# zehuichen123/Graph-DETR4D

Measured on AMD Instinct MI355X. Metric: decoder_samples_per_sec_900q_T4, higher is better.
Workload: dtype f32 (bf16x3 GEMMs)

## Files before the change

graph-detr4d_amd/_lib.py:

```python
import ctypes
import os
import threading

from . import switches

_HERE = os.path.dirname(os.path.abspath(__file__))
LIB_PATH = switches.path('GD4D_LIB_PATH') or os.path.join(_HERE, 'libgd4d.so')
ABI_VERSION = 56
PIXEL_MAJOR, HEAD_MAJOR = 0, 1

F32, BF16, F16 = 0, 1, 2
GATHER_REVERSED = 0x100

_c = ctypes
_vp, _i, _f = _c.c_void_p, _c.c_int, _c.c_float

SIGNATURES = {
    'gd4d_abi_version': (_i, []),
    'gd4d_error_string': (_c.c_char_p, [_i]),
    'gd4d_last_hip_error': (_c.c_char_p, []),
    'gd4d_trace_enable': (_i, [_vp]),
    'gd4d_cross_attn_fwd': (_i, [_vp, _vp, _vp, _vp, _vp, _vp, _vp, _vp, _f, _f, _vp, _vp, _vp,
                                 _i, _i, _i, _i, _i, _i, _i, _i, _i, _i, _vp, _vp]),
    'gd4d_pyramid_channels_last_fwd': (_i, [_vp, _vp, _vp, _i, _i, _i, _i, _i, _i, _vp]),
    'gd4d_cross_attn_agg_fwd': (_i, [_vp] * 8 + [_f, _f] + [_vp] * 4 + [_i] * 9 + [_vp] * 5),
    'gd4d_cross_attn_plan_bytes': (_c.c_size_t, [_i] * 5),
    'gd4d_cross_attn_plan_fwd': (_i, [_vp] * 6 + [_f, _f, _vp, _vp, _c.c_int64, _vp, _c.c_size_t, _vp, _vp, _vp] + [_i] * 7 + [_vp, _vp]),
    'gd4d_cross_attn_agg_sliced_fwd': (_i, [_vp, _c.c_int64, _vp, _vp] + [_i] * 8 + [_vp, _i, _i, _vp]),
    'gd4d_cross_attn_agg_items_fwd': (_i, [_vp, _vp, _vp, _c.c_int64, _c.c_int64, _vp, _vp, _vp] + [_i] * 8 + [_vp, _i, _i, _vp]),
    'gd4d_cross_attn_agg_items_coarse_fwd': (_i, [_vp, _vp, _vp, _c.c_int64, _c.c_int64, _vp, _vp, _vp, _vp, _vp, _vp] + [_i] * 8 + [_vp, _vp]),
    'gd4d_gather_slice_group': (_i, [_i]),
    'gd4d_gather_slice_group_get': (_i, []),
    'gd4d_gather_walk': (_i, [_i, _i, _i, _i, _vp, _vp]),
    'gd4d_gather_walk_dir': (_i, [_i, _i, _i, _i, _i, _vp, _vp]),
    'gd4d_chain_guest_bytes': (_c.c_size_t, []),
    'gd4d_value_proj_image_bytes': (_c.c_size_t, []),
    'gd4d_value_proj_image': (_i, [_vp, _vp, _vp, _vp]),
    'gd4d_value_proj_guest_fwd': (_i, [_vp, _i, _vp]),
    'gd4d_row_chain_guest_fwd': (_i, [_vp, _i, _vp, _i, _i, _vp, _vp]),
    'gd4d_row_chain_choice': (_i, [_vp, _i, _vp, _i, _i]),
    'gd4d_row_chain_choice_name': (_c.c_char_p, [_i]),
    'gd4d_row_chain_specialise': (_i, [_i]),
    'gd4d_row_chain_fill_fwd': (_i, [_vp, _i, _vp, _i, _i, _vp, _i, _vp, _vp, _i, _i, _i, _i, _i, _vp]),
    'gd4d_cross_attn_agg_items_count_fwd': (_i, [_vp, _vp, _vp, _c.c_int64, _c.c_int64, _vp, _vp, _vp] + [_i] * 8 + [_vp, _vp, _vp, _vp, _c.c_size_t, _vp]),
    'gd4d_pyramid_slice_planar_fwd': (_i, [_vp, _vp, _vp, _i, _i, _i, _i, _i, _i, _vp]),
    'gd4d_value_proj_heads_fwd': (_i, [_vp] * 5 + [_i, _i, _i, _vp]),
    'gd4d_value_proj_heads_bwd': (_i, [_vp] * 5 + [_i, _i, _i, _vp]),
    'gd4d_value_proj_heads_bwd_weight_workspace_bytes': (_c.c_size_t, []),
    'gd4d_value_proj_heads_bwd_weight': (_i, [_vp] * 6 + [_c.c_size_t, _i, _i, _i, _i, _vp]),
    'gd4d_value_proj_heads_bwd_weight_group': (_i, [_vp] * 6 + [_i, _vp, _c.c_size_t, _i, _i, _i, _vp]),
    'gd4d_cross_attn_dot_bytes': (_c.c_size_t, [_i] * 5),
    'gd4d_cross_attn_dot_sliced': (_i, [_vp, _c.c_int64, _vp, _vp, _vp, _c.c_size_t] + [_i] * 8 + [_vp, _vp]),
    'gd4d_cross_attn_dot_sliced_wgrad': (_i, [_vp, _c.c_int64, _vp, _vp, _vp, _c.c_size_t] + [_i] * 8 + [_vp] + [_vp] * 5 + [_i, _i, _vp]),
    'gd4d_cross_attn_plan_bwd': (_i, [_vp] * 6 + [_f, _f] + [_vp] * 9 + [_c.c_size_t, _vp] + [_i] * 7 + [_vp, _vp]),
    'gd4d_pyramid_grad_chunks': (_c.c_int64, [_vp, _i, _i]),
    'gd4d_pyramid_grad_slots_bytes': (_c.c_size_t, [_i] * 5),
    'gd4d_pyramid_grad_count': (_i, [_vp, _vp, _vp, _c.c_int64, _vp, _vp, _c.c_size_t] + [_i] * 6 + [_vp]),
    'gd4d_pyramid_grad_scan_workspace_bytes': (_c.c_size_t, [_c.c_int64]),
    'gd4d_pyramid_grad_scan': (_i, [_vp, _vp, _vp, _c.c_size_t, _c.c_int64, _vp]),
    'gd4d_pyramid_grad_fill': (_i, [_vp, _vp, _vp, _vp, _c.c_uint32, _vp] + [_i] * 5 + [_vp]),
    'gd4d_pyramid_grad_chunk_geometry': (_i, [_vp, _i, _i, _vp]),
    'gd4d_pyramid_grad_sort': (_i, [_vp] * 5 + [_c.c_int64, _vp]),
    'gd4d_pyramid_grad_reduce': (_i, [_vp] * 7 + [_i, _i, _i, _i, _vp]),
    'gd4d_query_order_fwd': (_i, [_vp, _vp, _vp, _i, _i, _vp]),
    'gd4d_refine_reference_order_fwd': (_i, [_vp, _vp, _vp, _vp, _vp, _i, _i, _i, _vp]),
    'gd4d_cross_attn_bwd': (_i, [_vp] * 8 + [_f, _f] + [_vp] * 6 + [_i] * 10 + [_vp, _vp, _c.c_size_t, _vp]),
    'gd4d_cross_attn_bwd_workspace_bytes': (_c.c_size_t, [_i] * 5),
    'gd4d_detr3d_fwd': (_i, [_vp, _vp, _vp, _vp, _vp, _vp, _f, _f, _vp, _vp, _vp,
# ... 220 lines not shown
```

graph-detr4d_amd/csrc/gd4d_cross_attn_sliced.hip:

```cpp
#include <stdlib.h>

#include <type_traits>

#include "gd4d_common.h"
#include "gd4d_cross_attn_shared.h"
#include "gd4d_cross_attn_sliced.h"
#include "gd4d_pyramid_count.h"

namespace gd4d {

GD4D_TRACE_UNIT(sliced)


struct PlanParams {
  CrossAttnParams c;
  PyramidGeom g;
  int* hdr;
  uint2* pair;
  int cap_t;
  float4* item;
  int cap_i;
  int both;
};

// ... 286 lines not shown
  if (grp - k * period == ca.every && k < ca.groups) {
    pyramid_grad_count_body(ca.hdr, ca.pair, ca.cap_t, HH, ca.BQ, ca.g, ca.count, ca.slots,
                            (k * 8 + (int)(blockIdx.x & 7)) * HH + (int)(threadIdx.x >> 6));
    return;
  }
  int pos, sl;
  if (!sliced_walk(ip.s, (int)blockIdx.x - 8 * min(k, ca.groups), pos, sl)) return;
  cross_attn_agg_items_body<HH, LT, VT, false>(ip, pos, sl, s_raw);
}

struct SpParams {
  const float* in[GD4D_MAX_LEVELS];
  int hw[GD4D_MAX_LEVELS];
  int start[GD4D_MAX_LEVELS];
  int tiles[GD4D_MAX_LEVELS];
  int tile_base[GD4D_MAX_LEVELS + 1];
  void* out;
  int R, L, S, total;
};

constexpr int SP_PX = 64, SP_C = 256, SP_PITCH = 260, SP_THREADS = 512;
constexpr int SP_LDS = 84 * 1024;

template <bool OUT_BF16>
__device__ __forceinline__ void sp_store4(void* base, size_t elem, float4 v) {
  if (OUT_BF16) {
    uint2 pk;
    pk.x = (unsigned)f32_to_bf16(v.x) | ((unsigned)f32_to_bf16(v.y) << 16);
    pk.y = (unsigned)f32_to_bf16(v.z) | ((unsigned)f32_to_bf16(v.w) << 16);
    *reinterpret_cast<uint2*>(static_cast<uint16_t*>(base) + elem) = pk;
  } else {
    *reinterpret_cast<float4*>(static_cast<float*>(base) + elem) = v;
  }
}

template <bool OUT_BF16, bool PERSISTENT>
__global__ __launch_bounds__(SP_THREADS) void pyramid_slice_planar_kernel(const SpParams p) {
  extern __shared__ __attribute__((aligned(16))) float s_tp[];
  const int tid = threadIdx.x, lane = tid & 63, wave = tid >> 6;
  trace_mark(g_trace_sliced, 4ull);
  float v[32];
  int npx = 0, ostart = 0, pix0 = 0, row = 0;
  auto load_tile = [&](int t) {
    const float* src = p.in[0];
    int hw = p.hw[0], tiles = p.tiles[0], tbase = 0, os = p.start[0];
#pragma unroll
// ... 11 lines not shown
  int t = blockIdx.x;
  if (t < p.total) load_tile(t);
  const size_t plane = (size_t)p.R * p.S * kSlice;
  while (t < p.total) {
    const int c_npx = npx, c_ostart = ostart, c_pix0 = pix0, c_row = row;
#pragma unroll
    for (int i = 0; i < 32; ++i) s_tp[lane * SP_PITCH + wave * 32 + i] = v[i];
    __syncthreads();
    const int tn = t + gridDim.x;
    if (PERSISTENT && tn < p.total) load_tile(tn);
    const size_t obase = (size_t)wave * plane + ((size_t)c_row * p.S + c_ostart + c_pix0) * kSlice;
#pragma unroll
    for (int i = 0; i < SP_PX / 8; ++i) {
      const int px = 8 * i + (lane >> 3);
      if (px < c_npx)
        sp_store4<OUT_BF16>(p.out, obase + (size_t)px * kSlice + (lane & 7) * 4,
                            *reinterpret_cast<const float4*>(&s_tp[px * SP_PITCH + wave * 32 + (lane & 7) * 4]));
    }
    if (!PERSISTENT) break;
    __syncthreads();
    t = tn;
  }
  trace_mark(g_trace_sliced, 0x84ull);
}

}

extern "C" void gd4d_trace_set_sliced(unsigned long long* p) { gd4d::trace_set_sliced(p); }

extern "C" size_t gd4d_cross_attn_plan_bytes(int B, int N, int Q, int Hh, int P) {
  if (B <= 0 || N <= 0 || Q <= 0 || Hh <= 0 || P <= 0) return 0;
  const size_t pairs = (size_t)B * Q * Hh * gd4d::plan_cap_t(N, P) * 64 * sizeof(uint2);
  return gd4d::plan_hdr_bytes(B, Q) + pairs;
}

namespace gd4d {
static int fill_plan_params(PlanParams& pp, const float* ref, const float* offsets, const float* attn_logits,
                            const float* cam_logits, const float* lidar2img, const double* pc_range, float img_h, float img_w,
                            const int32_t* level_hw, const int64_t* cam_stride_bytes, int64_t pix_stride_bytes, void* plan,
                            size_t plan_bytes, float* wsum, uint8_t* mask_out, float* uv_out, int B, int N, int Q, int Hh, int L, int P,
                            int flags, const int32_t* query_order);
}

extern "C" int gd4d_cross_attn_plan_fwd(const float* ref, const float* offsets, const float* attn_logits,
                                        const float* cam_logits, const float* lidar2img, const double* pc_range,
                                        float img_h, float img_w, const int32_t* level_hw, const int64_t* cam_stride_bytes,
// ... 309 lines not shown
extern "C" int gd4d_cross_attn_agg_items_count_fwd(const void* const* level_ptrs, const int32_t* level_hw,
                                                   const int64_t* cam_stride_bytes, int64_t pix_stride_bytes,
                                                   int64_t slice_stride_bytes, const void* plan_items, float* agg, float* wsum, int B,
                                                   int N, int Q, int Hh, int C, int L, int P, int feats_dtype,
                                                   const int32_t* query_order, const void* plan_pairs, int32_t* count, void* slots,
                                                   size_t slots_bytes, void* stream) {
  using namespace gd4d;
  if (!plan_pairs || !count || !slots || !level_hw || !cam_stride_bytes) return GD4D_EINVAL;
  if (B <= 0 || N <= 0 || Q <= 0 || Hh <= 0 || L <= 0) return GD4D_EINVAL;
  if ((P != kPoints && P != 8) || L > 4 || N > 64 || B > 16 || Hh > kPlanHdr) return GD4D_EUNSUPPORTED;
  if (slots_bytes < (size_t)B * Q * Hh * plan_cap_t(N, P) * 64 * sizeof(uint2)) return GD4D_EWORKSPACE;
  CountArgs ca{};
  if (int rc = fill_chunks(ca.g, level_hw, cam_stride_bytes, pix_stride_bytes, B * N, L)) return rc;
  ca.hdr = static_cast<const int*>(plan_pairs);
  ca.pair = reinterpret_cast<const uint2*>(static_cast<const char*>(plan_pairs) + plan_hdr_bytes(B, Q));
  ca.count = count;
  ca.slots = static_cast<uint2*>(slots);
  ca.cap_t = plan_cap_t(N, P);
  ca.BQ = B * Q;
  return items_fwd_impl(level_ptrs, level_hw, cam_stride_bytes, pix_stride_bytes, slice_stride_bytes, plan_items, agg, wsum, B, N, Q, Hh,
                        C, L, P, feats_dtype, query_order, 0, 8, stream, &ca);
}

extern "C" int gd4d_pyramid_slice_planar_fwd(const void* const* feats, const int32_t* level_hw, void* out, int R, int C,
                                             int L, int in_dtype, int out_dtype, int max_cus, void* stream) {
  using namespace gd4d;
  if (!feats || !level_hw || !out || R <= 0 || C <= 0 || L <= 0) return GD4D_EINVAL;
  if (C != SP_C || L > GD4D_MAX_LEVELS || in_dtype != GD4D_F32) return GD4D_EUNSUPPORTED;
  if (out_dtype != GD4D_F32 && out_dtype != GD4D_BF16) return GD4D_EUNSUPPORTED;
  if (!aligned16(out)) return GD4D_EALIGN;
  SpParams p{};
  int s = 0, base = 0;
  for (int l = 0; l < L; ++l) {
    if (!feats[l] || level_hw[2 * l] <= 0 || level_hw[2 * l + 1] <= 0) return GD4D_EINVAL;
    const int hw = level_hw[2 * l] * level_hw[2 * l + 1];
    p.in[l] = static_cast<const float*>(feats[l]); p.hw[l] = hw; p.start[l] = s; p.tiles[l] = (hw + SP_PX - 1) / SP_PX;
    p.tile_base[l] = base;
    s += hw;
    base += R * p.tiles[l];
  }
  for (int l = L; l <= GD4D_MAX_LEVELS; ++l) p.tile_base[l] = base;
  for (int l = L; l < GD4D_MAX_LEVELS; ++l) { p.tiles[l] = 1; p.hw[l] = 1; }
  p.out = out; p.R = R; p.L = L; p.S = s; p.total = base;
  hipStream_t st = static_cast<hipStream_t>(stream);
  const bool ob = out_dtype == GD4D_BF16;
  const size_t tile_lds = (size_t)SP_PX * SP_PITCH * sizeof(float);
  auto go = [&](auto kern, int blocks, size_t lds) -> int {
    if (!allow_dynamic_lds(reinterpret_cast<const void*>(kern), (int)lds)) return GD4D_ELAUNCH;
    hipLaunchKernelGGL(kern, dim3(blocks), dim3(SP_THREADS), lds, st, p);
    return check_launch();
  };
  if (max_cus > 0) {
    const int blocks = max_cus < base ? max_cus : base;
    return ob ? go(pyramid_slice_planar_kernel<true, true>, blocks, SP_LDS) : go(pyramid_slice_planar_kernel<false, true>, blocks, SP_LDS);
  }
  return ob ? go(pyramid_slice_planar_kernel<true, false>, base, tile_lds) : go(pyramid_slice_planar_kernel<false, false>, base, tile_lds);
}
```

graph-detr4d_amd/csrc/gd4d_request.hip:

```cpp
#include <string.h>

#include <new>
#include <vector>

#include "gd4d_common.h"

namespace {

struct Step {
  gd4d_request_step s;
  std::vector<gd4d_chain_op> prog_a, prog_b;
  gd4d_chain_guest guest;
  std::vector<gd4d_request_patch> patches;
  std::vector<uint64_t> table[GD4D_REQ_TABLES];
};

bool is_chain(int kind) { return kind == GD4D_REQ_ROW_CHAIN || kind == GD4D_REQ_ROW_CHAIN2 || kind == GD4D_REQ_ROW_CHAIN_GUEST; }

struct Shape {
  const char* name;
  int ptrs, tables;
};

const Shape* shape_of(int kind) {
  static const Shape shapes[] = {
      {nullptr, 0, 0},
      {"gd4d_row_chain_fwd", 0, 0},
      {"gd4d_row_chain2_fwd", 0, 0},
      {"gd4d_row_chain_guest_fwd", 0, 0},
      {"gd4d_mha_core_fwd", 5, 0},
      {"gd4d_mha_core_presplit_fwd", 5, 0},
      {"gd4d_cross_attn_plan_fwd", 10, 3},
      {"gd4d_cross_attn_agg_items_coarse_fwd", 5, 5},
      {"gd4d_cross_attn_agg_items_fwd", 4, 3},
      {"gd4d_cross_attn_agg_sliced_fwd", 3, 1},
      {"gd4d_pyramid_slice_planar_fwd", 1, 2},
      {"gd4d_value_proj_guest_fwd", 0, 0},
      {"gd4d_query_order_fwd", 2, 1},
      {"hipEventRecord", 0, 0},
      {"hipStreamWaitEvent", 0, 0},
      {"hipMemcpyAsync", 2, 0},
  };
  if (kind < GD4D_REQ_ROW_CHAIN || kind > GD4D_REQ_COPY) return nullptr;
  return &shapes[kind];
}

int64_t table_need(const gd4d_request_step& s, int k) {
  const int64_t L = s.kind == GD4D_REQ_SLICE_PLANAR ? s.i[2] : s.kind == GD4D_REQ_PLAN ? s.i[4] : s.i[5];
  switch (s.kind) {
    case GD4D_REQ_PLAN: return k == 0 ? 48 : k == 1 ? 8 * L : 8 * L;
    case GD4D_REQ_AGG_COARSE: return k == 0 ? 8 * L : k == 1 ? 8 * L : k == 2 ? 8 * L : 16;
    case GD4D_REQ_AGG_ITEMS: return 8 * L;
    case GD4D_REQ_AGG_SLICED: return 8 * L;
    case GD4D_REQ_SLICE_PLANAR: return 8 * L;
    case GD4D_REQ_QUERY_ORDER: return 48;
  }
  return 0;
}

}

struct gd4d_decoder_request {
  std::vector<Step> steps;
  std::vector<hipEvent_t> events;
  hipEvent_t join = nullptr;
  int nbindings = 0;
  bool uses_side = false;
};

namespace {

int validate(const gd4d_request_step* steps, int nsteps, int nbindings) {
  if (steps == nullptr || nsteps <= 0 || nsteps > GD4D_REQ_MAX_STEPS || nbindings < 0) return GD4D_EINVAL;
  bool recorded[GD4D_REQ_MAX_EVENTS] = {};
  for (int n = 0; n < nsteps; ++n) {
    const gd4d_request_step& s = steps[n];
    const Shape* sh = shape_of(s.kind);
    if (sh == nullptr || (s.side != 0 && s.side != 1) || s.npatches < 0 || (s.npatches > 0 && s.patches == nullptr)) return GD4D_EINVAL;
    for (int k = 0; k < sh->ptrs; ++k)
      if (s.p[k].binding >= nbindings) return GD4D_EINVAL;
    if (s.kind == GD4D_REQ_PLAN && (s.fbind[0] >= nbindings || s.fbind[1] >= nbindings)) return GD4D_EINVAL;
    if (is_chain(s.kind)) {
      if (s.prog_a == nullptr || s.nops_a <= 0 || s.nops_a > GD4D_CHAIN_MAX_OPS) return GD4D_EINVAL;
      const bool two = s.kind == GD4D_REQ_ROW_CHAIN2 || (s.kind == GD4D_REQ_ROW_CHAIN_GUEST && s.nops_b != 0);
      if (two && (s.prog_b == nullptr || s.nops_b <= 0 || s.nops_a + s.nops_b > GD4D_CHAIN_MAX_OPS)) return GD4D_EINVAL;
      if (s.i[0] <= 0) return GD4D_EINVAL;
    }
    if ((s.kind == GD4D_REQ_ROW_CHAIN_GUEST || s.kind == GD4D_REQ_VALUE_PROJ_GUEST) && s.guest == nullptr) return GD4D_EINVAL;
    for (int k = 0; k < sh->tables; ++k) {
      const int64_t need = table_need(s, k);
      if (s.table[k] == nullptr || need <= 0 || s.table_bytes[k] < need || s.table_bytes[k] > (1 << 20)) return GD4D_EINVAL;
    }
    if (s.kind == GD4D_REQ_EVENT_RECORD || s.kind == GD4D_REQ_STREAM_WAIT) {
      if (s.event < 0 || s.event >= GD4D_REQ_MAX_EVENTS) return GD4D_EINVAL;
      if (s.kind == GD4D_REQ_EVENT_RECORD) recorded[s.event] = true;
      else if (!recorded[s.event]) return GD4D_EINVAL;
    }
    if (s.kind == GD4D_REQ_COPY && s.l[0] <= 0) return GD4D_EINVAL;
    for (int k = 0; k < s.npatches; ++k) {
      const gd4d_request_patch& pt = s.patches[k];
// ... 41 lines not shown
      return gd4d_mha_core_presplit_fwd(F(0), P(1), P(2), F(3), i[0], i[1], i[2], i[3], i[4], s.l[0], s.l[1], P(4), i[5], s.f[0], nullptr,
                                        0.f, nullptr, stream);
    case GD4D_REQ_PLAN: {
      const float img_h = s.fbind[0] >= 0 ? static_cast<float>(b[s.fbind[0]].scalar) : s.f[0];
      const float img_w = s.fbind[1] >= 0 ? static_cast<float>(b[s.fbind[1]].scalar) : s.f[1];
      return gd4d_cross_attn_plan_fwd(F(0), F(1), F(2), F(3), F(4), static_cast<const double*>(T(0)), img_h, img_w,
                                      static_cast<const int32_t*>(T(1)), static_cast<const int64_t*>(T(2)), s.l[0], P(5),
                                      static_cast<size_t>(s.l[1]), F(6), static_cast<uint8_t*>(P(7)), F(8), i[0], i[1], i[2], i[3], i[4],
                                      i[5], i[6], static_cast<const int32_t*>(P(9)), stream);
    }
    case GD4D_REQ_AGG_COARSE:
      return gd4d_cross_attn_agg_items_coarse_fwd(static_cast<const void* const*>(T(0)), static_cast<const int32_t*>(T(1)),
                                                  static_cast<const int64_t*>(T(2)), s.l[0], s.l[1], static_cast<const void* const*>(T(3)),
                                                  static_cast<const int64_t*>(T(4)), P(0), F(1), F(2), F(3), i[0], i[1], i[2], i[3], i[4],
                                                  i[5], i[6], i[7], static_cast<const int32_t*>(P(4)), stream);
    case GD4D_REQ_AGG_ITEMS:
      return gd4d_cross_attn_agg_items_fwd(static_cast<const void* const*>(T(0)), static_cast<const int32_t*>(T(1)),
                                           static_cast<const int64_t*>(T(2)), s.l[0], s.l[1], P(0), F(1), F(2), i[0], i[1], i[2], i[3], i[4],
                                           i[5], i[6], i[7], static_cast<const int32_t*>(P(3)), i[8], i[9], stream);
    case GD4D_REQ_AGG_SLICED:
      return gd4d_cross_attn_agg_sliced_fwd(static_cast<const void* const*>(T(0)), s.l[0], P(0), F(1), i[0], i[1], i[2], i[3], i[4], i[5],
                                            i[6], i[7], static_cast<const int32_t*>(P(2)), i[8], i[9], stream);
    case GD4D_REQ_SLICE_PLANAR:
      return gd4d_pyramid_slice_planar_fwd(static_cast<const void* const*>(T(0)), static_cast<const int32_t*>(T(1)), P(0), i[0], i[1], i[2],
                                           i[3], i[4], i[5], stream);
    case GD4D_REQ_VALUE_PROJ_GUEST: return gd4d_value_proj_guest_fwd(&st.guest, i[0], stream);
    case GD4D_REQ_QUERY_ORDER:
      return gd4d_query_order_fwd(F(0), static_cast<const double*>(T(0)), static_cast<int32_t*>(P(1)), i[0], i[1], stream);
    case GD4D_REQ_EVENT_RECORD:
    case GD4D_REQ_STREAM_WAIT:
    case GD4D_REQ_COPY: {
      hipError_t e = s.kind == GD4D_REQ_EVENT_RECORD  ? hipEventRecord(req->events[s.event], stream)
                     : s.kind == GD4D_REQ_STREAM_WAIT ? hipStreamWaitEvent(stream, req->events[s.event], 0)
                                                      : hipMemcpyAsync(P(0), P(1), static_cast<size_t>(s.l[0]), hipMemcpyDeviceToDevice, stream);
      if (e != hipSuccess) {
        gd4d::set_last_hip_error(e);
        return GD4D_ELAUNCH;
      }
      return GD4D_OK;
    }
  }
  return GD4D_EINVAL;
}

void release(gd4d_decoder_request* req) {
  for (hipEvent_t e : req->events)
    if (e != nullptr) (void)hipEventDestroy(e);
  if (req->join != nullptr) (void)hipEventDestroy(req->join);
  delete req;
}

}

extern "C" size_t gd4d_request_step_bytes(void) { return sizeof(gd4d_request_step); }

extern "C" int gd4d_decoder_request_create(const gd4d_request_step* steps, int nsteps, int nbindings, gd4d_decoder_request** out) {
  if (out == nullptr) return GD4D_EINVAL;
  *out = nullptr;
  const int code = validate(steps, nsteps, nbindings);
  if (code != GD4D_OK) return code;
  gd4d_decoder_request* req = new (std::nothrow) gd4d_decoder_request();
  if (req == nullptr) return GD4D_EINVAL;
  req->nbindings = nbindings;
  req->steps.resize(nsteps);
  int nevents = 0;
  for (int n = 0; n < nsteps; ++n) {
    Step& st = req->steps[n];
    st.s = steps[n];
    gd4d_request_step& s = st.s;
    const Shape* sh = shape_of(s.kind);
    memset(&st.guest, 0, sizeof(st.guest));
    if (is_chain(s.kind)) {
      st.prog_a.assign(s.prog_a, s.prog_a + s.nops_a);
      if (s.prog_b != nullptr && s.nops_b > 0 && s.kind != GD4D_REQ_ROW_CHAIN) st.prog_b.assign(s.prog_b, s.prog_b + s.nops_b);
      else s.nops_b = 0;
    }
    if (s.guest != nullptr && (s.kind == GD4D_REQ_ROW_CHAIN_GUEST || s.kind == GD4D_REQ_VALUE_PROJ_GUEST)) st.guest = *s.guest;
    if (s.npatches > 0) st.patches.assign(s.patches, s.patches + s.npatches);
    for (int k = 0; k < sh->tables; ++k) {
      st.table[k].assign(static_cast<size_t>((s.table_bytes[k] + 7) / 8), 0);
      memcpy(st.table[k].data(), s.table[k], static_cast<size_t>(s.table_bytes[k]));
    }
    s.prog_a = s.prog_b = nullptr;
    s.guest = nullptr;
    s.patches = nullptr;
    for (int k = 0; k < GD4D_REQ_TABLES; ++k) s.table[k] = nullptr;
    if (s.kind == GD4D_REQ_EVENT_RECORD && s.event + 1 > nevents) nevents = s.event + 1;
    if (s.side != 0) req->uses_side = true;
  }
  req->events.assign(nevents, nullptr);
  for (int n = 0; n < nevents + (req->uses_side ? 1 : 0); ++n) {
    hipEvent_t e = nullptr;
    hipError_t err = hipEventCreateWithFlags(&e, hipEventDisableTiming);
// ... 15 lines not shown
  if (req->uses_side && (side_stream == nullptr || side_stream == stream)) return GD4D_EINVAL;
  hipStream_t main_s = static_cast<hipStream_t>(stream), side_s = static_cast<hipStream_t>(side_stream);
  bool side_touched = false;
  for (Step& st : req->steps) {
    const bool side = st.s.side != 0;
    const int code = issue(req, st, bindings, side ? side_s : main_s);
    if (code != GD4D_OK) {
      if (side_touched && hipEventRecord(req->join, side_s) == hipSuccess) (void)hipStreamWaitEvent(main_s, req->join, 0);
      return code;
    }
    side_touched = side_touched || side;
  }
  return GD4D_OK;
}

extern "C" int gd4d_decoder_request_destroy(gd4d_decoder_request* req) {
  if (req == nullptr) return GD4D_EINVAL;
  release(req);
  return GD4D_OK;
}

extern "C" const char* gd4d_decoder_request_describe(const gd4d_decoder_request* req, int i) {
  if (req == nullptr || i < 0 || i >= static_cast<int>(req->steps.size())) return nullptr;
  return shape_of(req->steps[i].s.kind)->name;
}
```

graph-detr4d_amd/functional.py:

```python
import numpy as np

import torch

from . import _lib, ops, switches


def wants_grad(module, *tensors):
    if not torch.is_grad_enabled():
        return False
    if any(t is not None and torch.is_tensor(t) and t.requires_grad for t in tensors):
        return True
    return module is not None and any(p.requires_grad for p in module.parameters())


def require_inference(*tensors):
    if torch.is_grad_enabled() and any(t is not None and t.requires_grad for t in tensors):
        raise NotImplementedError(
            'graph-detr4d_amd: this entry point has no backward - call it under torch.no_grad()')


def main_grad(t, rows=None):
    m = getattr(t, '_gd4d_main_grad', None) if t is not None else None
    if m is None or rows is None:
        return m
# ... 500 lines not shown
    ev = torch.cuda.Event()
    ev.record(stream)
    return ev


def _wait_event(stream, event):
    rec = _lib.recorder()
    if rec is None:
        stream.wait_event(event)
    else:
        rec.wait_event(stream, event)


LATE_VALUES_KEY = '_gd4d_late_values'


class LateValues:

    def __init__(self, value, dtype=torch.float32, coarse_for=None):
        dev = value[0].device
        self.value = value
        self.main = torch.cuda.current_stream(dev)
        self.shapes = [(int(v.shape[-2]), int(v.shape[-1])) for v in value]
        self.cl = self.pyramid = self.event = self.src = None
        self.copy_dtype = torch.float32
        self.coarse = self.coarse_src = self.coarse_first = None
        self.partial = False
        self.project_late = False
        self.waited = set()
        if all(ops.PyramidView.is_channels_last_level(v) for v in value) and len({v.dtype for v in value}) == 1 \
                and value[0].dtype in (torch.float32, torch.bfloat16):
            self.mode, self.side = 'sliced', None
            self.pyramid = ops.PyramidView.channels_last_levels(list(value))
            if coarse_for and self.coarse_setup(coarse_for):
                self.side = _companion_stream(_SIDE_STREAMS, dev)
                _wait_stream(self.side, self.main)
                with torch.cuda.stream(self.side):
                    self._project_first(coarse_for[0])
                    self.event = _record_event(self.side)
                self.coarse.rows.record_stream(self.main)
            return
        self.mode = switches.choice('GD4D_AGG')
        if self.mode == 'rows' and value[0].shape[0] != 1:
            self.mode = 'sliced'
        self.side = _companion_stream(_SIDE_STREAMS, dev)
        _wait_stream(self.side, self.main)
        with torch.cuda.stream(self.side):
            env = switches.integer('GD4D_COPY_CUS')
            cus = torch.cuda.get_device_properties(dev).multi_processor_count
            copy_cus = env if env is not None else max(8, (cus * 3 // 4) // 8 * 8)
            src = [v.contiguous() for v in value]
            self.src, self.copy_cus, self.copy_dtype = src, copy_cus, dtype
            if self.mode == 'sliced':
                if coarse_for and self.coarse_setup(coarse_for):
                    if switches.choice('GD4D_FIRST_PROJ') == 'main':
                        self.coarse_first, self.project_late = coarse_for[0], True
                    else:
                        self._project_first(coarse_for[0])
                    self.coarse.rows.record_stream(self.main)
                    self.partial = True
                if self.partial:
                    self.cl, _ = ops.pyramid_slice_planar_fwd(src[:2], max_cus=copy_cus, out_dtype=dtype)
                    fine = ops.PyramidView.slice_planar(self.cl, self.shapes[:2])
                    self.pyramid = ops.PyramidView([self.cl], fine.ptrs + fine.ptrs[:1] * 2, self.shapes, fine.cam_stride + fine.cam_stride[:1] * 2,
                                                   fine.pix_stride, fine.slice_stride, fine.dtype, fine.rows)
                else:
                    self.cl, _ = ops.pyramid_slice_planar_fwd(src, max_cus=copy_cus, out_dtype=dtype)
                    self.pyramid = ops.PyramidView.slice_planar(self.cl, self.shapes)
            else:
                self.cl, _ = ops.pyramid_channels_last_fwd(src, max_cus=copy_cus, out_dtype=dtype)
            self.event = _record_event(self.side)
        self.cl.record_stream(self.main)

    def _project_first(self, module):
        ops.value_proj_guest_fwd(self.coarse_guest(module))
        self.coarse_first = module

    def take_first(self, module):
        hit, self.coarse_first = self.coarse_first is module, None
        return hit

    def _ensure_full(self):
        if not self.partial:
            return
        self._wait_copy()
        self.cl, _ = ops.pyramid_slice_planar_fwd(self.src, max_cus=0, out_dtype=self.copy_dtype)
        self.pyramid = ops.PyramidView.slice_planar(self.cl, self.shapes)
        self.partial = False

    @staticmethod
# ... 130 lines not shown
```

graph-detr4d_amd/fused_decoder.py:

```python
import ctypes
import weakref

import torch
import torch.nn as nn

from . import _lib
from . import functional as Fn
from . import ops
from . import switches
from .deform3d_cross_attn import Deform3DCrossAttn
from .transformer_layers import FFN, MultiheadAttention

ORDER = ('self_attn', 'norm', 'cross_attn', 'norm', 'ffn', 'norm')
OFFSETS_EXACT = True


def _plain_reg_branch(branch, c):
    if not isinstance(branch, nn.Sequential) or len(branch) % 2 == 0:
        return None
    lins = []
    for i, m in enumerate(branch):
        if i % 2 == 0:
            if not isinstance(m, nn.Linear) or m.in_features != c or (i + 1 < len(branch) and m.out_features != c):
                return None
# ... 506 lines not shown
    ref = query_pos.transpose(0, 1)[..., :3] if reference_points is None else reference_points
    if not takes_single_stream_loop(decoder, query, value, ref, reg_branches, masks, query_pos):
        return None
    ok, mask = _request_mask(masks)
    cross = [l.attentions[1] for l in decoder.layers]
    if not ok or query.device.index != torch.cuda.current_device() or not Fn.LateValues.applicable(cross, value) \
            or query_pos.dtype != torch.float32 or query_pos.shape != query.shape or query_pos.stride(-1) != 1 or query.stride(-1) != 1 \
            or not (all(v.is_contiguous() for v in value) or all(ops.PyramidView.is_channels_last_level(v) for v in value)):
        return None
    return (mask,)


def request_forward(decoder, query, reference_points, reg_branches, kwargs):
    covered = kwargs.get(REQUEST_OK_KEY)
    if covered is None:
        covered = request_covers(decoder, query, reference_points, reg_branches, kwargs)
    if covered is None or not reference_points.is_contiguous() or reference_points.dtype != torch.float32:
        return None
    mask, value, query_pos, img_metas = covered[0], kwargs['value'], kwargs['query_pos'], kwargs['img_metas']
    dev = query.device
    key = (dev.index, torch.cuda.current_stream(dev).cuda_stream, Fn.slot_key(dev), tuple(query.shape), query.stride(), query_pos.stride(),
           tuple((tuple(v.shape), v.stride(), v.dtype) for v in value), None if mask is None else (tuple(mask.shape), mask.dtype),
           reg_branches is None, decoder.return_intermediate, len(img_metas), switches.schedule_key(),
           bool(ops.ALL_EXACT[0]), ops.handoff_enabled(dev, 'GD4D_POS_ENCODER'), decoder.layers[0].attentions[1].value_dtype)
    table = _PROGRAMS.get(decoder)
    if table is None:
        table = _PROGRAMS[decoder] = {}
    prog = table.get(key)
    if prog is None or not prog.valid(reg_branches):
        if prog is not None:
            table.pop(key).close()
        while len(table) >= 8:
            table.pop(next(iter(table))).close()
        prog = table[key] = RequestProgram(decoder, query, query_pos, reference_points, reg_branches, value, img_metas, mask)
    outs, refs = prog.run(query, query_pos, reference_points, value, img_metas, mask)
    if decoder.return_intermediate:
        return outs, refs
    return outs[0], refs[0]
```

graph-detr4d_amd/ops.py:

```python
import ctypes
import functools
import inspect
import weakref

import torch

from . import _lib, switches

F32, I32, U8 = torch.float32, torch.int32, torch.uint8


def _dev(t, name, dtype=None):
    if not t.is_cuda:
        raise _lib.Gd4dError(f'{name} must live on the GPU (no CPU fallback in graph-detr4d_amd)')
    if dtype is not None and t.dtype != dtype:
        raise TypeError(f'{name} must be {dtype}, got {t.dtype}')
    if not t.is_contiguous():
        raise ValueError(f'{name} must be contiguous')
    return ctypes.c_void_p(t.data_ptr())


def _opt(t, name, dtype=F32):
    return None if t is None else _dev(t, name, dtype)

# ... 91 lines not shown
    b, q = ref.shape[0], ref.shape[1]
    n = lidar2img.shape[1]
    hh, p = num_heads, offsets.shape[3]
    nl = len(level_hw)
    c = feats_cl.shape[-1]
    if feats_cl.shape[0] != b * n or feats_cl.shape[1] != sum(h * w for h, w in level_hw):
        raise ValueError(f'feats_cl shape {tuple(feats_cl.shape)} inconsistent with B*N={b * n}, levels {level_hw}')
    if offsets.numel() != b * q * hh * p * 3 or attn_logits.numel() != b * q * hh * nl * p or cam_logits.numel() != b * q * n:
        raise ValueError('offsets / attn_logits / cam_logits have the wrong number of elements')
    fused = vp_weight is not None
    agg = None if fused else torch.empty(b, q, hh, c, device=ref.device, dtype=F32)
    wsum = None if fused else torch.empty(b, q, hh, device=ref.device, dtype=F32)
    out = torch.empty(b, q, c, device=ref.device, dtype=F32) if fused else None
    mask = torch.empty(b, n, q, hh, p, device=ref.device, dtype=U8) if want_mask else None
    uv = torch.empty(b, n, q, hh, p, 2, device=ref.device, dtype=F32) if want_uv else None
    _call('gd4d_cross_attn_agg_fwd', _dev(feats_cl, 'feats_cl'), _levels(level_hw),
          *_camera_args(ref, offsets, attn_logits, cam_logits, lidar2img, pc_range, img_h, img_w), _opt(agg, 'agg', None),
          _opt(wsum, 'wsum', None), _opt(mask, 'mask', None), _opt(uv, 'uv', None), b, n, q, hh, c, nl, p, _value_dtype(feats_cl),
          1 if raw_cam_weights else 0, _order_ptr(query_order, b * q), _opt(vp_weight, 'vp_weight'),
          _opt(vp_bias, 'vp_bias') if fused else None, _opt(out, 'out', None))
    return _asked((out,) if fused else (agg, wsum), mask, uv, bare=False)


def pyramid_slice_planar_fwd(feats, out=None, max_cus=0, out_dtype=torch.float32):
    fl = [f.reshape(-1, *f.shape[-3:]) for f in feats]
    r, c = fl[0].shape[0], fl[0].shape[1]
    level_hw = [(int(f.shape[-2]), int(f.shape[-1])) for f in fl]
    s = sum(h * w for h, w in level_hw)
    if any(f.shape[0] != r or f.shape[1] != c for f in fl):
        raise ValueError('feature levels disagree in rows / channels')
    if c != 256:
        raise ValueError('the slice-planar copy is built for 256 channels')
    if out is None:
        out = torch.empty(8, r, s, 32, device=fl[0].device, dtype=out_dtype)
    ptrs = _ptrs(fl, 'feats')
    lv = _levels(level_hw)
    _call('gd4d_pyramid_slice_planar_fwd', ptrs, lv, _dev(out, 'out'), r, c, len(fl), _lib.F32, _value_dtype(out), int(max_cus))
    return out, level_hw


class PyramidView:

    def __init__(self, tensors, ptrs, level_hw, cam_stride, pix_stride, slice_stride, dtype, rows):
        self.tensors, self.ptrs, self.level_hw = tensors, ptrs, [tuple(int(x) for x in hw) for hw in level_hw]
        self.cam_stride, self.pix_stride, self.slice_stride = [int(x) for x in cam_stride], int(pix_stride), int(slice_stride)
        self.dtype, self.rows = dtype, int(rows)

    @property
    def device(self):
        return self.tensors[0].device

    @staticmethod
    def _starts(level_hw):
        out, s = [], 0
        for h, w in level_hw:
            out.append(s)
            s += h * w
        return out, s

    @classmethod
    def slice_planar(cls, sp, level_hw):
# ... 2203 lines not shown
                                     special={4: 'lidar2img'}, fbind=['img_h', 'img_w'], f=[img_h, img_w], l=[pix, plan_bytes],
                                     i=[b, n, q, hh, nl, p, flags], tables=[(rng, False), (lv, False), (cs, False)]))
        return 0

    def gd4d_cross_attn_agg_items_coarse_fwd(self, ptrs, lv, cs, pix, sl, pp, pcs, plan, agg, wsum, pagg, b, n, q, hh, c, nl, p, dt, order,
                                             stream):
        self.pending.append(_Pending(REQ_AGG_COARSE, self._side(stream), p=[plan, agg, wsum, pagg, order], l=[pix, sl],
                                     i=[b, n, q, hh, c, nl, p, dt],
                                     tables=[(ptrs, True), (lv, False), (cs, False), (pp, True), (pcs, False)]))
        return 0

    def gd4d_cross_attn_agg_items_fwd(self, ptrs, lv, cs, pix, sl, plan, agg, wsum, b, n, q, hh, c, nl, p, dt, order, lo, cnt, stream):
        self.pending.append(_Pending(REQ_AGG_ITEMS, self._side(stream), p=[plan, agg, wsum, order], l=[pix, sl],
                                     i=[b, n, q, hh, c, nl, p, dt, lo, cnt], tables=[(ptrs, True), (lv, False), (cs, False)]))
        return 0

    def gd4d_cross_attn_agg_sliced_fwd(self, ptrs, sl, plan, agg, b, n, q, hh, c, nl, p, dt, order, lo, cnt, stream):
        self.pending.append(_Pending(REQ_AGG_SLICED, self._side(stream), p=[plan, agg, order], l=[sl],
                                     i=[b, n, q, hh, c, nl, p, dt, lo, cnt], tables=[(ptrs, True)]))
        return 0

    def gd4d_pyramid_slice_planar_fwd(self, feats, lv, out, r, c, nl, in_dt, out_dt, max_cus, stream):
        self.pending.append(_Pending(REQ_SLICE_PLANAR, self._side(stream), p=[out], i=[r, c, nl, in_dt, out_dt, max_cus],
                                     tables=[(feats, True), (lv, False)]))
        return 0

    def gd4d_query_order_fwd(self, ref, rng, order, b, q, stream):
        self.pending.append(_Pending(REQ_QUERY_ORDER, self._side(stream), p=[ref, order], i=[b, q], tables=[(rng, False)]))
        return 0

    def steps(self, bindings, named):
        exact = {t.data_ptr(): k for k, t in bindings.items()}
        extents = [(*tensor_extent(t), k) for k, t in bindings.items()]

        def find(addr):
            if addr == 0:
                return None
            if addr in exact:
                return exact[addr], 0
            for lo, hi, k in extents:
                if lo <= addr < hi:
                    return k, addr - lo
            return None

        keep, arr = [], (RequestStep * len(self.pending))()
        for s, pd in zip(arr, self.pending):
# ... 883 lines not shown
```

include/gd4d.h:

```cpp
#ifndef GD4D_H_
#define GD4D_H_

#include <stddef.h>
#include <stdint.h>

#ifdef __cplusplus
extern "C" {
#endif

#define GD4D_ABI_VERSION 56

enum { GD4D_F32 = 0, GD4D_BF16 = 1, GD4D_F16 = 2 };

enum { GD4D_LAYOUT_PIXEL_MAJOR = 0, GD4D_LAYOUT_HEAD_MAJOR = 1 };

enum { GD4D_VP_PRECISION_F32 = 0, GD4D_VP_PRECISION_BF16 = 1 };

enum {
  GD4D_OK = 0,
  GD4D_EINVAL = -1,
  GD4D_EUNSUPPORTED = -2,
  GD4D_EALIGN = -3,
  GD4D_ELAUNCH = -4,
  GD4D_EWORKSPACE = -5
// ... 42 lines not shown

int gd4d_gather_slice_group(int ns);
int gd4d_gather_slice_group_get(void);
int gd4d_gather_walk(int BQ, int blk, int ns, int block, int* pos, int* group);

#define GD4D_GATHER_REVERSED 0x100
int gd4d_gather_walk_dir(int BQ, int blk, int ns, int reversed, int block, int* pos, int* group);

int gd4d_cross_attn_agg_items_count_fwd(const void* const* level_ptrs, const int32_t* level_hw, const int64_t* cam_stride_bytes,
                                        int64_t pix_stride_bytes, int64_t slice_stride_bytes, const void* plan_items, float* agg,
                                        float* wsum, int B, int N, int Q, int Hh, int C, int L, int P, int feats_dtype,
                                        const int32_t* query_order, const void* plan_pairs, int32_t* count, void* slots,
                                        size_t slots_bytes, void* stream);
int gd4d_cross_attn_plan_fwd(const float* ref, const float* offsets, const float* attn_logits, const float* cam_logits,
                             const float* lidar2img, const double* pc_range, float img_h, float img_w,
                             const int32_t* level_hw, const int64_t* cam_stride_bytes, int64_t pix_stride_bytes, void* plan,
                             size_t plan_bytes, float* wsum, uint8_t* mask_out, float* uv_out, int B, int N, int Q, int Hh,
                             int L, int P, int flags, const int32_t* query_order, void* stream);
int gd4d_cross_attn_agg_sliced_fwd(const void* const* level_ptrs, int64_t slice_stride_bytes, const void* plan, float* agg,
                                   int B, int N, int Q, int Hh, int C, int L, int P, int feats_dtype,
                                   const int32_t* query_order, int slice_lo, int slice_n, void* stream);
int gd4d_pyramid_slice_planar_fwd(const void* const* feats, const int32_t* level_hw, void* out, int R, int C, int L,
                                  int in_dtype, int out_dtype, int max_cus, void* stream);

int gd4d_value_proj_heads_bwd(const float* grad_out, const float* weight, const float* bias, float* grad_agg, float* beta,
                              int M, int Hh, int C, void* stream);
size_t gd4d_value_proj_heads_bwd_weight_workspace_bytes(void);
int gd4d_value_proj_heads_bwd_weight(const float* grad_out, const float* agg, const float* wsum, float* grad_weight,
                                     float* grad_bias, void* workspace, size_t workspace_bytes, int M, int Hh, int C,
                                     int accumulate, void* stream);
int gd4d_value_proj_heads_bwd_weight_group(const void* const* grad_out, const void* const* agg, const void* const* wsum,
                                           void* const* grad_weight, void* const* grad_bias, const int32_t* rows, int count,
                                           void* workspace, size_t workspace_bytes, int Hh, int C, int accumulate, void* stream);
size_t gd4d_cross_attn_dot_bytes(int B, int N, int Q, int Hh, int P);
int gd4d_cross_attn_dot_sliced(const void* const* level_ptrs, int64_t slice_stride_bytes, const void* plan,
                               const float* grad_agg, void* dpart, size_t dpart_bytes, int B, int N, int Q, int Hh, int C, int L,
                               int P, int feats_dtype, const int32_t* query_order, void* stream);

int gd4d_cross_attn_dot_sliced_wgrad(const void* const* level_ptrs, int64_t slice_stride_bytes, const void* plan,
                                     const float* grad_agg, void* dpart, size_t dpart_bytes, int B, int N, int Q, int Hh, int C,
                                     int L, int P, int feats_dtype, const int32_t* query_order, const void* const* x,
                                     const void* const* grad_y, void* const* grad_w, void* const* grad_b, const int32_t* dims,
                                     int count, int accumulate, void* stream);

int gd4d_cross_attn_plan_bwd(const float* ref, const float* offsets, const float* attn_logits, const float* cam_logits,
                             const float* lidar2img, const double* pc_range, float img_h, float img_w, const int32_t* level_hw,
// ... 535 lines not shown
```

Before: 716.7.

## Add atomic work-queue variant of planar pyramid slice copy kernel

Adds a dynamically scheduled version of the pyramid slice-planar copy, where persistent workgroups claim tiles through a global atomic counter instead of a fixed grid stride. The last workgroup to arrive resets the counter. It is enabled by default in sliced mode through a per-device queue buffer, and the request/graph machinery dispatches to it. The aim is to balance load across the reduced set of copy CUs that share the device with concurrent decoder work. The cost is an extra atomic per tile and reliance on the counter reset being correct across calls.

```diff
diff --git a/graph-detr4d_amd/_lib.py b/graph-detr4d_amd/_lib.py
--- a/graph-detr4d_amd/_lib.py
+++ b/graph-detr4d_amd/_lib.py
@@ -44,6 +44,8 @@
     'gd4d_row_chain_fill_fwd': (_i, [_vp, _i, _vp, _i, _i, _vp, _i, _vp, _vp, _i, _i, _i, _i, _i, _vp]),
     'gd4d_cross_attn_agg_items_count_fwd': (_i, [_vp, _vp, _vp, _c.c_int64, _c.c_int64, _vp, _vp, _vp] + [_i] * 8 + [_vp, _vp, _vp, _vp, _c.c_size_t, _vp]),
     'gd4d_pyramid_slice_planar_fwd': (_i, [_vp, _vp, _vp, _i, _i, _i, _i, _i, _i, _vp]),
+    'gd4d_pyramid_slice_planar_queue_fwd': (_i, [_vp, _vp, _vp, _vp, _i, _i, _i, _i, _i, _i, _vp]),
+    'gd4d_slice_copy_tile': (_i, [_vp, _i, _i, _i, _vp, _vp, _vp, _vp]),
     'gd4d_value_proj_heads_fwd': (_i, [_vp] * 5 + [_i, _i, _i, _vp]),
     'gd4d_value_proj_heads_bwd': (_i, [_vp] * 5 + [_i, _i, _i, _vp]),
     'gd4d_value_proj_heads_bwd_weight_workspace_bytes': (_c.c_size_t, []),
diff --git a/graph-detr4d_amd/csrc/gd4d_cross_attn_sliced.hip b/graph-detr4d_amd/csrc/gd4d_cross_attn_sliced.hip
--- a/graph-detr4d_amd/csrc/gd4d_cross_attn_sliced.hip
+++ b/graph-detr4d_amd/csrc/gd4d_cross_attn_sliced.hip
@@ -332,6 +332,16 @@
 constexpr int SP_PX = 64, SP_C = 256, SP_PITCH = 260, SP_THREADS = 512;
 constexpr int SP_LDS = 84 * 1024;
 
+#ifndef SP_TRACE_TAIL
+#define SP_TRACE_TAIL 0
+#endif
+__device__ __forceinline__ void sp_trace_tail() {
+#if SP_TRACE_TAIL
+  unsigned long long* t = g_trace_sliced;
+  if (t && threadIdx.x == 0) atomicMax(t + 2 + 2 * t[1], (unsigned long long)__builtin_amdgcn_s_memrealtime());
+#endif
+}
+
 template <bool OUT_BF16>
 __device__ __forceinline__ void sp_store4(void* base, size_t elem, float4 v) {
   if (OUT_BF16) {
@@ -389,6 +399,79 @@
     t = tn;
   }
   trace_mark(g_trace_sliced, 0x84ull);
+  if (PERSISTENT) sp_trace_tail();
+}
+
+constexpr int SP_Q_ARRIVE = 32;
+
+__device__ __forceinline__ void sp_queue_arrive(unsigned* q) {
+  if (threadIdx.x == 0 && atomicAdd(q + SP_Q_ARRIVE, 1u) == gridDim.x - 1) {
+    __hip_atomic_store(q, 0u, __ATOMIC_RELAXED, __HIP_MEMORY_SCOPE_AGENT);
+    __hip_atomic_store(q + SP_Q_ARRIVE, 0u, __ATOMIC_RELAXED, __HIP_MEMORY_SCOPE_AGENT);
+  }
+}
+
+__host__ __device__ __forceinline__ int sp_tile_at(const SpParams& p, int t, int& row, int& pix0, int& npx) {
+  int l = 0;
+#pragma unroll
+  for (int k = 1; k < GD4D_MAX_LEVELS; ++k)
+    if (k < p.L && t >= p.tile_base[k]) l = k;
+  const int rel = t - p.tile_base[l];
+  row = rel / p.tiles[l];
+  pix0 = (rel - row * p.tiles[l]) * SP_PX;
+  npx = p.hw[l] - pix0 < SP_PX ? p.hw[l] - pix0 : SP_PX;
+  return l;
+}
+
+template <bool OUT_BF16>
+__global__ __launch_bounds__(SP_THREADS) void pyramid_slice_planar_queue_kernel(const SpParams p, unsigned* const q) {
+  extern __shared__ __attribute__((aligned(16))) float s_tp[];
+  int* const s_next = reinterpret_cast<int*>(s_tp + SP_PX * SP_PITCH);
+  const int tid = threadIdx.x, lane = tid & 63, wave = tid >> 6;
+  trace_mark(g_trace_sliced, 4ull);
+  float v[32];
+  int npx = 0, ostart = 0, pix0 = 0, row = 0;
+  auto load_tile = [&](int t) {
+    const int l = sp_tile_at(p, t, row, pix0, npx);
+    const int hw = p.hw[l];
+    ostart = p.start[l];
+    const float* gp = p.in[l] + ((size_t)row * SP_C + wave * 32) * hw + pix0 + min(lane, npx - 1);
+#pragma unroll
+    for (int i = 0; i < 32; ++i) v[i] = gp[(size_t)i * hw];
+  };
+  const int total = p.total;
+  int t = blockIdx.x;
+  unsigned pend = 0;
+  if (t < total) {
+    if (tid == 0) pend = atomicAdd(q, 1u);
+    load_tile(t);
+  }
+  const size_t plane_elems = (size_t)p.R * p.S * kSlice;
+  while (t < total) {
+    const int c_npx = npx, c_ostart = ostart, c_pix0 = pix0, c_row = row;
+#pragma unroll
+    for (int i = 0; i < 32; ++i) s_tp[lane * SP_PITCH + wave * 32 + i] = v[i];
+    if (tid == 0) *s_next = (int)min(pend + gridDim.x, (unsigned)total);
+    __syncthreads();
+    const int tn = __builtin_amdgcn_readfirstlane(*s_next);
+    if (tn < total) {
+      if (tid == 0) pend = atomicAdd(q, 1u);
+      load_tile(tn);
+    }
+    const size_t obase = (size_t)wave * plane_elems + ((size_t)c_row * p.S + c_ostart + c_pix0) * kSlice;
+#pragma unroll
+    for (int i = 0; i < SP_PX / 8; ++i) {
+      const int px = 8 * i + (lane >> 3);
+      if (px < c_npx)
+        sp_store4<OUT_BF16>(p.out, obase + (size_t)px * kSlice + (lane & 7) * 4,
+                            *reinterpret_cast<const float4*>(&s_tp[px * SP_PITCH + wave * 32 + (lane & 7) * 4]));
+    }
+    __syncthreads();
+    t = tn;
+  }
+  sp_queue_arrive(q);
+  trace_mark(g_trace_sliced, 0x84ull);
+  sp_trace_tail();
 }
 
 }
@@ -744,6 +827,61 @@
                         C, L, P, feats_dtype, query_order, 0, 8, stream, &ca);
 }
 
+namespace gd4d {
+static int fill_sp_params(SpParams& p, const void* const* feats, const int32_t* level_hw, void* out, int R, int L) {
+  int64_t s = 0, base = 0;
+  for (int l = 0; l < L; ++l) {
+    if ((feats && !feats[l]) || level_hw[2 * l] <= 0 || level_hw[2 * l + 1] <= 0) return GD4D_EINVAL;
+    const int64_t hw = (int64_t)level_hw[2 * l] * level_hw[2 * l + 1];
+    if (hw > 0x7fffffffll - SP_PX) return GD4D_EUNSUPPORTED;
+    p.in[l] = feats ? static_cast<const float*>(feats[l]) : nullptr;
+    p.hw[l] = (int)hw; p.start[l] = (int)s; p.tiles[l] = (int)((hw + SP_PX - 1) / SP_PX);
+    p.tile_base[l] = (int)base;
+    s += hw;
+    base += (int64_t)R * p.tiles[l];
+    if (s > 0x7fffffffll || base > 0x7fffffffll) return GD4D_EUNSUPPORTED;
+  }
+  for (int l = L; l <= GD4D_MAX_LEVELS; ++l) p.tile_base[l] = (int)base;
+  for (int l = L; l < GD4D_MAX_LEVELS; ++l) { p.tiles[l] = 1; p.hw[l] = 1; }
+  p.out = out; p.R = R; p.L = L; p.S = (int)s; p.total = (int)base;
+  return GD4D_OK;
+}
+}
+
+extern "C" int gd4d_slice_copy_tile(const int32_t* level_hw, int R, int L, int tile, int* level, int* row, int* pix0, int* npx) {
+  using namespace gd4d;
+  if (!level_hw || R <= 0 || L <= 0 || L > GD4D_MAX_LEVELS) return GD4D_EINVAL;
+  SpParams p{};
+  if (int rc = fill_sp_params(p, nullptr, level_hw, nullptr, R, L)) return rc;
+  int l = -1, r = -1, x = -1, n = -1;
+  if (tile >= 0 && tile < p.total) l = sp_tile_at(p, tile, r, x, n);
+  if (level) *level = l;
+  if (row) *row = r;
+  if (pix0) *pix0 = x;
+  if (npx) *npx = n;
+  return p.total;
+}
+
+extern "C" int gd4d_pyramid_slice_planar_queue_fwd(const void* const* feats, const int32_t* level_hw, void* out, void* queue, int R,
+                                                   int C, int L, int in_dtype, int out_dtype, int workgroups, void* stream) {
+  using namespace gd4d;
+  if (!feats || !level_hw || !out || !queue || R <= 0 || C <= 0 || L <= 0 || workgroups <= 0) return GD4D_EINVAL;
+  if (C != SP_C || L > GD4D_MAX_LEVELS || in_dtype != GD4D_F32 || workgroups > 65536) return GD4D_EUNSUPPORTED;
+  if (out_dtype != GD4D_F32 && out_dtype != GD4D_BF16) return GD4D_EUNSUPPORTED;
+  if (!aligned16(out) || (reinterpret_cast<uintptr_t>(queue) & 127u)) return GD4D_EALIGN;
+  SpParams p{};
+  if (int rc = fill_sp_params(p, feats, level_hw, out, R, L)) return rc;
+  for (int l = L; l < GD4D_MAX_LEVELS; ++l) p.in[l] = p.in[0];
+  hipStream_t st = static_cast<hipStream_t>(stream);
+  unsigned* q = static_cast<unsigned*>(queue);
+  auto go = [&](auto kern) -> int {
+    if (!allow_dynamic_lds(reinterpret_cast<const void*>(kern), SP_LDS)) return GD4D_ELAUNCH;
+    hipLaunchKernelGGL(kern, dim3(workgroups), dim3(SP_THREADS), SP_LDS, st, p, q);
+    return check_launch();
+  };
+  return out_dtype == GD4D_BF16 ? go(pyramid_slice_planar_queue_kernel<true>) : go(pyramid_slice_planar_queue_kernel<false>);
+}
+
 extern "C" int gd4d_pyramid_slice_planar_fwd(const void* const* feats, const int32_t* level_hw, void* out, int R, int C,
                                              int L, int in_dtype, int out_dtype, int max_cus, void* stream) {
   using namespace gd4d;
@@ -752,18 +890,8 @@
   if (out_dtype != GD4D_F32 && out_dtype != GD4D_BF16) return GD4D_EUNSUPPORTED;
   if (!aligned16(out)) return GD4D_EALIGN;
   SpParams p{};
-  int s = 0, base = 0;
-  for (int l = 0; l < L; ++l) {
-    if (!feats[l] || level_hw[2 * l] <= 0 || level_hw[2 * l + 1] <= 0) return GD4D_EINVAL;
-    const int hw = level_hw[2 * l] * level_hw[2 * l + 1];
-    p.in[l] = static_cast<const float*>(feats[l]); p.hw[l] = hw; p.start[l] = s; p.tiles[l] = (hw + SP_PX - 1) / SP_PX;
-    p.tile_base[l] = base;
-    s += hw;
-    base += R * p.tiles[l];
-  }
-  for (int l = L; l <= GD4D_MAX_LEVELS; ++l) p.tile_base[l] = base;
-  for (int l = L; l < GD4D_MAX_LEVELS; ++l) { p.tiles[l] = 1; p.hw[l] = 1; }
-  p.out = out; p.R = R; p.L = L; p.S = s; p.total = base;
+  if (int rc = fill_sp_params(p, feats, level_hw, out, R, L)) return rc;
+  const int base = p.total;
   hipStream_t st = static_cast<hipStream_t>(stream);
   const bool ob = out_dtype == GD4D_BF16;
   const size_t tile_lds = (size_t)SP_PX * SP_PITCH * sizeof(float);
diff --git a/graph-detr4d_amd/csrc/gd4d_request.hip b/graph-detr4d_amd/csrc/gd4d_request.hip
--- a/graph-detr4d_amd/csrc/gd4d_request.hip
+++ b/graph-detr4d_amd/csrc/gd4d_request.hip
@@ -45,6 +45,11 @@
   return &shapes[kind];
 }
 
+const Shape* shape_of(const gd4d_request_step& s) {
+  static const Shape queue = {"gd4d_pyramid_slice_planar_queue_fwd", 2, 2};
+  return s.kind == GD4D_REQ_SLICE_PLANAR && s.i[6] != 0 ? &queue : shape_of(s.kind);
+}
+
 int64_t table_need(const gd4d_request_step& s, int k) {
   const int64_t L = s.kind == GD4D_REQ_SLICE_PLANAR ? s.i[2] : s.kind == GD4D_REQ_PLAN ? s.i[4] : s.i[5];
   switch (s.kind) {
@@ -75,7 +80,7 @@
   bool recorded[GD4D_REQ_MAX_EVENTS] = {};
   for (int n = 0; n < nsteps; ++n) {
     const gd4d_request_step& s = steps[n];
-    const Shape* sh = shape_of(s.kind);
+    const Shape* sh = shape_of(s);
     if (sh == nullptr || (s.side != 0 && s.side != 1) || s.npatches < 0 || (s.npatches > 0 && s.patches == nullptr)) return GD4D_EINVAL;
     for (int k = 0; k < sh->ptrs; ++k)
       if (s.p[k].binding >= nbindings) return GD4D_EINVAL;
@@ -163,6 +168,9 @@
       return gd4d_cross_attn_agg_sliced_fwd(static_cast<const void* const*>(T(0)), s.l[0], P(0), F(1), i[0], i[1], i[2], i[3], i[4], i[5],
                                             i[6], i[7], static_cast<const int32_t*>(P(2)), i[8], i[9], stream);
     case GD4D_REQ_SLICE_PLANAR:
+      if (i[6] != 0)
+        return gd4d_pyramid_slice_planar_queue_fwd(static_cast<const void* const*>(T(0)), static_cast<const int32_t*>(T(1)), P(0), P(1), i[0],
+                                                   i[1], i[2], i[3], i[4], i[5], stream);
       return gd4d_pyramid_slice_planar_fwd(static_cast<const void* const*>(T(0)), static_cast<const int32_t*>(T(1)), P(0), i[0], i[1], i[2],
                                            i[3], i[4], i[5], stream);
     case GD4D_REQ_VALUE_PROJ_GUEST: return gd4d_value_proj_guest_fwd(&st.guest, i[0], stream);
@@ -209,7 +217,7 @@
     Step& st = req->steps[n];
     st.s = steps[n];
     gd4d_request_step& s = st.s;
-    const Shape* sh = shape_of(s.kind);
+    const Shape* sh = shape_of(s);
     memset(&st.guest, 0, sizeof(st.guest));
     if (is_chain(s.kind)) {
       st.prog_a.assign(s.prog_a, s.prog_a + s.nops_a);
@@ -271,5 +279,5 @@
 
 extern "C" const char* gd4d_decoder_request_describe(const gd4d_decoder_request* req, int i) {
   if (req == nullptr || i < 0 || i >= static_cast<int>(req->steps.size())) return nullptr;
-  return shape_of(req->steps[i].s.kind)->name;
-}
+  return shape_of(req->steps[i].s)->name;
+}
diff --git a/graph-detr4d_amd/functional.py b/graph-detr4d_amd/functional.py
--- a/graph-detr4d_amd/functional.py
+++ b/graph-detr4d_amd/functional.py
@@ -546,7 +546,7 @@
         self.value = value
         self.main = torch.cuda.current_stream(dev)
         self.shapes = [(int(v.shape[-2]), int(v.shape[-1])) for v in value]
-        self.cl = self.pyramid = self.event = self.src = None
+        self.cl = self.pyramid = self.event = self.src = self.queue = None
         self.copy_dtype = torch.float32
         self.coarse = self.coarse_src = self.coarse_first = None
         self.partial = False
@@ -569,6 +569,8 @@
             self.mode = 'sliced'
         self.side = _companion_stream(_SIDE_STREAMS, dev)
         _wait_stream(self.side, self.main)
+        if self.mode == 'sliced' and ops.slice_copy_queue():
+            self.queue = ops.slice_copy_queue_words(dev, slot_key(dev))
         with torch.cuda.stream(self.side):
             env = switches.integer('GD4D_COPY_CUS')
             cus = torch.cuda.get_device_properties(dev).multi_processor_count
@@ -584,12 +586,12 @@
                     self.coarse.rows.record_stream(self.main)
                     self.partial = True
                 if self.partial:
-                    self.cl, _ = ops.pyramid_slice_planar_fwd(src[:2], max_cus=copy_cus, out_dtype=dtype)
+                    self.cl, _ = ops.pyramid_slice_planar_fwd(src[:2], max_cus=copy_cus, out_dtype=dtype, queue=self.queue)
                     fine = ops.PyramidView.slice_planar(self.cl, self.shapes[:2])
                     self.pyramid = ops.PyramidView([self.cl], fine.ptrs + fine.ptrs[:1] * 2, self.shapes, fine.cam_stride + fine.cam_stride[:1] * 2,
                                                    fine.pix_stride, fine.slice_stride, fine.dtype, fine.rows)
                 else:
-                    self.cl, _ = ops.pyramid_slice_planar_fwd(src, max_cus=copy_cus, out_dtype=dtype)
+                    self.cl, _ = ops.pyramid_slice_planar_fwd(src, max_cus=copy_cus, out_dtype=dtype, queue=self.queue)
                     self.pyramid = ops.PyramidView.slice_planar(self.cl, self.shapes)
             else:
                 self.cl, _ = ops.pyramid_channels_last_fwd(src, max_cus=copy_cus, out_dtype=dtype)
diff --git a/graph-detr4d_amd/fused_decoder.py b/graph-detr4d_amd/fused_decoder.py
--- a/graph-detr4d_amd/fused_decoder.py
+++ b/graph-detr4d_amd/fused_decoder.py
@@ -552,7 +552,8 @@
     key = (dev.index, torch.cuda.current_stream(dev).cuda_stream, Fn.slot_key(dev), tuple(query.shape), query.stride(), query_pos.stride(),
            tuple((tuple(v.shape), v.stride(), v.dtype) for v in value), None if mask is None else (tuple(mask.shape), mask.dtype),
            reg_branches is None, decoder.return_intermediate, len(img_metas), switches.schedule_key(),
-           bool(ops.ALL_EXACT[0]), ops.handoff_enabled(dev, 'GD4D_POS_ENCODER'), decoder.layers[0].attentions[1].value_dtype)
+           bool(ops.ALL_EXACT[0]), ops.handoff_enabled(dev, 'GD4D_POS_ENCODER'), decoder.layers[0].attentions[1].value_dtype,
+           ops.slice_copy_queue())
     table = _PROGRAMS.get(decoder)
     if table is None:
         table = _PROGRAMS[decoder] = {}
diff --git a/graph-detr4d_amd/ops.py b/graph-detr4d_amd/ops.py
--- a/graph-detr4d_amd/ops.py
+++ b/graph-detr4d_amd/ops.py
@@ -137,7 +137,7 @@
     return _asked((out,) if fused else (agg, wsum), mask, uv, bare=False)
 
 
-def pyramid_slice_planar_fwd(feats, out=None, max_cus=0, out_dtype=torch.float32):
+def pyramid_slice_planar_fwd(feats, out=None, max_cus=0, out_dtype=torch.float32, queue=None):
     fl = [f.reshape(-1, *f.shape[-3:]) for f in feats]
     r, c = fl[0].shape[0], fl[0].shape[1]
     level_hw = [(int(f.shape[-2]), int(f.shape[-1])) for f in fl]
@@ -150,8 +150,44 @@
         out = torch.empty(8, r, s, 32, device=fl[0].device, dtype=out_dtype)
     ptrs = _ptrs(fl, 'feats')
     lv = _levels(level_hw)
+    if queue is not None and max_cus > 0:
+        if queue.dtype != I32 or queue.numel() < SLICE_COPY_QUEUE_WORDS or not queue.is_contiguous():
+            raise ValueError(f'queue: {SLICE_COPY_QUEUE_WORDS} contiguous int32 words')
+        _call('gd4d_pyramid_slice_planar_queue_fwd', ptrs, lv, _dev(out, 'out'), _dev(queue, 'queue', I32), r, c, len(fl), _lib.F32,
+              _value_dtype(out), int(max_cus))
+        return out, level_hw
     _call('gd4d_pyramid_slice_planar_fwd', ptrs, lv, _dev(out, 'out'), r, c, len(fl), _lib.F32, _value_dtype(out), int(max_cus))
     return out, level_hw
+
+
+SLICE_COPY_QUEUE_WORDS = 64
+_SLICE_COPY_QUEUES = {}
+_SLICE_COPY_QUEUE = [True]
+
+
+def slice_copy_queue(on=None):
+    was = _SLICE_COPY_QUEUE[0]
+    if on is not None:
+        _SLICE_COPY_QUEUE[0] = bool(on)
+    return was
+
+
+def slice_copy_queue_words(device, slot_key):
+    device = torch.device(device)
+    key = (device.index, slot_key)
+    buf = _SLICE_COPY_QUEUES.get(key)
+    if buf is None:
+        if torch.cuda.is_current_stream_capturing():
+            return torch.zeros(SLICE_COPY_QUEUE_WORDS, device=device, dtype=I32)
+        buf = _SLICE_COPY_QUEUES[key] = torch.zeros(SLICE_COPY_QUEUE_WORDS, device=device, dtype=I32)
+    return buf
+
+
+def slice_copy_tile(level_hw, rows, tile):
+    out = [ctypes.c_int(-1) for _ in range(4)]
+    total = _lib.load().gd4d_slice_copy_tile(_levels(level_hw), int(rows), len(level_hw), int(tile), *[ctypes.byref(o) for o in out])
+    _lib.check(total if total < 0 else 0, 'gd4d_slice_copy_tile')
+    return (total,) + tuple(o.value for o in out)
 
 
 class PyramidView:
@@ -2401,6 +2437,11 @@
 
     def gd4d_pyramid_slice_planar_fwd(self, feats, lv, out, r, c, nl, in_dt, out_dt, max_cus, stream):
         self.pending.append(_Pending(REQ_SLICE_PLANAR, self._side(stream), p=[out], i=[r, c, nl, in_dt, out_dt, max_cus],
+                                     tables=[(feats, True), (lv, False)]))
+        return 0
+
+    def gd4d_pyramid_slice_planar_queue_fwd(self, feats, lv, out, queue, r, c, nl, in_dt, out_dt, workgroups, stream):
+        self.pending.append(_Pending(REQ_SLICE_PLANAR, self._side(stream), p=[out, queue], i=[r, c, nl, in_dt, out_dt, workgroups, 1],
                                      tables=[(feats, True), (lv, False)]))
         return 0
 
diff --git a/include/gd4d.h b/include/gd4d.h
--- a/include/gd4d.h
+++ b/include/gd4d.h
@@ -88,6 +88,11 @@
                                    const int32_t* query_order, int slice_lo, int slice_n, void* stream);
 int gd4d_pyramid_slice_planar_fwd(const void* const* feats, const int32_t* level_hw, void* out, int R, int C, int L,
                                   int in_dtype, int out_dtype, int max_cus, void* stream);
+
+#define GD4D_SLICE_COPY_QUEUE_BYTES 256
+int gd4d_pyramid_slice_planar_queue_fwd(const void* const* feats, const int32_t* level_hw, void* out, void* queue, int R, int C, int L,
+                                        int in_dtype, int out_dtype, int workgroups, void* stream);
+int gd4d_slice_copy_tile(const int32_t* level_hw, int R, int L, int tile, int* level, int* row, int* pix0, int* npx);
 
 int gd4d_value_proj_heads_bwd(const float* grad_out, const float* weight, const float* bias, float* grad_agg, float* beta,
                               int M, int Hh, int C, void* stream);
```

Result: no change. 722.1 (median of 6 runs) (+0.8%).
